# OpenVisualCloud/SVT-VP9

Measured on AMD Instinct MI355X. Metric: hot-path frames/sec (+ Mpixels/sec): block-level DSP path (picture analysis + ME + inter prediction from reconstructed references + DCT/quant/recon + deblock + reference padding), 3840x2160p60 yuv420p enc-mode 8; no mode decision, no entropy coding -- not encoded frames, higher is better.
Workload: dtype u8

## Files before the change

include/svtvp9_hip.h:

```cpp
#ifndef SVTVP9_HIP_H
#define SVTVP9_HIP_H

#include <stddef.h>
#include <stdint.h>

#ifdef __cplusplus
extern "C" {
#endif

typedef enum svt_hip_status {
    SVT_HIP_OK                 = 0,
    SVT_HIP_ERR_BAD_PARAMETER  = -1,
    SVT_HIP_ERR_NO_RESOURCES   = -2,
    SVT_HIP_ERR_DEVICE         = -3,
    SVT_HIP_ERR_UNSUPPORTED    = -4
} svt_hip_status;

typedef struct svt_hip_ctx svt_hip_ctx;


#define SVT_ME_PU_COUNT 85
#define SVT_SB_SIZE 64

typedef struct svt_plane {
// ... 54 lines not shown
    int16_t         x_mv_l0, y_mv_l0, x_mv_l1, y_mv_l1;
    svt_me_dist_dir distortion_direction[3];
    uint8_t         total_me_candidate_index;
    uint8_t         pad_[7];
} svt_me_pu_result;

int32_t svt_hip_sb_count(int32_t pic_width, int32_t pic_height);

int32_t svt_hip_input_resolution(int32_t pic_width, int32_t pic_height);

typedef struct svt_me_picture_config {
    int32_t pic_width, pic_height;
    int32_t enc_mode;
    int32_t tune;
    int32_t frame_rate;
    int32_t num_ref_lists;
    int32_t temporal_layer_index;
    int32_t hierarchical_levels;
    int32_t is_used_as_reference;
    int32_t same_ref_poc;
    int32_t rate_control_mode;
} svt_me_picture_config;

int32_t svt_hip_me_params_derive(svt_me_params *p, const svt_me_picture_config *cfg);

int32_t svt_hip_me_params_preset(svt_me_params *p, int32_t pic_width, int32_t pic_height, int32_t enc_mode,
                                 int32_t tune, int32_t num_ref_lists, int32_t temporal_layer_index,
                                 int32_t hierarchical_levels);

int32_t svt_hip_me_kernel_instance(const svt_me_params *p);
int32_t svt_hip_me_last_instance(const svt_hip_ctx *ctx);
int32_t svt_hip_me_lds_bytes(const svt_me_params *p, int32_t compact);
int32_t svt_hip_ctx_set_intra_workgroups(svt_hip_ctx *ctx, int32_t n);
int32_t svt_hip_ctx_warm(svt_hip_ctx *ctx);
int32_t svt_hip_ctx_warm_scratch(svt_hip_ctx *ctx, int32_t scratch_bytes);
int32_t svt_hip_me_params_same_launch(const svt_me_params *a, const svt_me_params *b);

int32_t svt_hip_ctx_create(svt_hip_ctx **ctx, int32_t device_ordinal);
int32_t svt_hip_ctx_create_on_stream(svt_hip_ctx **ctx, int32_t device_ordinal, void *hip_stream);
int32_t svt_hip_ctx_create_cu_mask(svt_hip_ctx **ctx, int32_t device, const uint32_t *cu_mask, int32_t mask_words);
void *svt_hip_ctx_stream(svt_hip_ctx *ctx);
void    svt_hip_ctx_destroy(svt_hip_ctx *ctx);
int32_t svt_hip_ctx_synchronize(svt_hip_ctx *ctx);
const char *svt_hip_last_error(void);
float   svt_hip_last_kernel_ms(svt_hip_ctx *ctx);

int32_t svt_hip_mem_alloc(svt_hip_ctx *ctx, size_t bytes, void **d_ptr);
void    svt_hip_mem_free(svt_hip_ctx *ctx, void *d_ptr);
int32_t svt_hip_mem_upload_2d(svt_hip_ctx *ctx, void *d_dst, size_t dst_stride, const void *src, size_t src_stride, size_t width_bytes,
                              size_t rows);
int32_t svt_hip_mem_download(svt_hip_ctx *ctx, void *dst, const void *d_src, size_t bytes);
int32_t svt_hip_mem_upload_2d_async(svt_hip_ctx *ctx, void *d_dst, size_t dst_stride, const void *src, size_t src_stride, size_t width_bytes,
                                    size_t rows);
int32_t svt_hip_mem_upload_planes_async(svt_hip_ctx *ctx, int32_t n_planes, void *const *d_dst, const size_t *dst_stride, const void *const *src,
                                        const size_t *src_stride, const size_t *width_bytes, const size_t *rows);
int32_t svt_hip_mem_upload_2d_direct(svt_hip_ctx *ctx, void *d_dst, size_t dst_stride, const void *src, size_t src_stride, size_t width_bytes,
                                     size_t rows);
int32_t svt_hip_mem_upload_wait(svt_hip_ctx *ctx);
void    svt_hip_host_unregister_all(void);
void    svt_hip_host_registry_retain(void);
void    svt_hip_host_registry_release(void);
int32_t svt_hip_ctx_marker_record(svt_hip_ctx *ctx, uint64_t *marker);
int32_t svt_hip_ctx_marker_query(svt_hip_ctx *ctx, uint64_t marker);
int32_t svt_hip_ctx_marker_wait(svt_hip_ctx *ctx, uint64_t marker);
int32_t svt_hip_mem_set(svt_hip_ctx *ctx, void *d_dst, int32_t value, size_t bytes);

// ... 459 lines not shown
```

svt-vp9_amd/binding.py:

```python
import ctypes as C
import os

import numpy as np

HERE = os.path.dirname(os.path.abspath(__file__))
LIB_PATH = os.environ.get("SVT_HIP_LIB") or os.path.join(HERE, "libsvtvp9_hip.so")

SVT_ME_PU_COUNT = 85


class Plane(C.Structure):
    _fields_ = [("buf", C.c_void_p), ("stride", C.c_int32), ("origin_x", C.c_int32), ("origin_y", C.c_int32),
                ("width", C.c_int32), ("height", C.c_int32)]


class PaPicture(C.Structure):
    _fields_ = [("full", Plane), ("quarter", Plane), ("sixteenth", Plane)]


class MeParams(C.Structure):
    _fields_ = [(n, C.c_uint8) for n in (
        "num_ref_lists", "temporal_layer_index", "hierarchical_levels", "enable_hme_flag",
        "enable_hme_level_0_flag", "enable_hme_level_1_flag", "enable_hme_level_2_flag", "cu8x8_mode",
        "cu16x16_mode", "same_ref_poc", "rate_control_mode", "fractional_search_method",
# ... 126 lines not shown
assert BOOL_TABLES_DTYPE.itemsize == 576 * 3 + 255 * 8 + 6 * 14
BOOL_SEGMENT_DTYPE = np.dtype([("first", "<u4"), ("count", "<u4"), ("kind", "<u4")])
BOOL_MAX_PER_TOKEN = 22
BOOL_SIZE_OVERFLOW = 0xFFFFFFFF
BOOL_MAX_STREAMS = 32


class BoolStream(C.Structure):
    _fields_ = [("d_tokens", C.c_void_p), ("d_bools", C.c_void_p), ("d_segments", C.c_void_p), ("d_n_tokens", C.c_void_p), ("n_segments", C.c_uint32),
                ("n_tokens", C.c_uint32), ("max_bools", C.c_uint32), ("capacity", C.c_uint32), ("d_bytes", C.c_void_p), ("d_size", C.c_void_p)]

OIS_BLOCK_DTYPE = np.dtype([("sad", "<u4"), ("uv_sad", "<u4"), ("mode", "u1"), ("uv_mode", "u1"), ("pad", "u1", (2,))])
assert OIS_BLOCK_DTYPE.itemsize == 12
OIS_PER_SB = 340
OIS_NONE = 0xFFFFFFFF

EXPORTS = [
    "svt_hip_sb_count", "svt_hip_input_resolution", "svt_hip_me_params_derive", "svt_hip_me_params_preset", "svt_hip_ctx_create", "svt_hip_ctx_create_on_stream", "svt_hip_ctx_create_cu_mask", "svt_hip_ctx_stream",
    "svt_hip_ctx_destroy", "svt_hip_ctx_synchronize", "svt_hip_last_error", "svt_hip_last_kernel_ms",
    "svt_hip_mem_alloc", "svt_hip_mem_free", "svt_hip_mem_upload_2d", "svt_hip_mem_upload_2d_async", "svt_hip_mem_upload_planes_async", "svt_hip_mem_download", "svt_hip_mem_set",
    "svt_hip_ctx_marker_record", "svt_hip_ctx_marker_query", "svt_hip_ctx_marker_wait", "svt_hip_minigop_split",
    "svt_hip_me_picture_device", "svt_hip_me_batch_device", "svt_hip_me_batch_layers_device", "svt_hip_me_picture", "svt_hip_sad_loop_batch_device",
    "svt_hip_me_zz_sad_device", "svt_hip_me_similar_collocated", "svt_hip_me_sb_stats_device", "svt_hip_pa_prepare_batch_device", "svt_hip_pa_mean_variance_device",
    "svt_hip_quant_tables_init", "svt_hip_tq_batch_device", "svt_hip_tq_batch_dist_device", "svt_hip_tq_rd_batch_device", "svt_hip_tq_rd_batch_multi_device", "svt_hip_rate_scan4x4_table", "svt_hip_tq_batch", "svt_hip_lf_thresh_init", "svt_hip_lf_level_from_q",
    "svt_hip_lf_frame_device", "svt_hip_lf_batch_device", "svt_hip_lf_frame", "svt_hip_lf_build_masks",
    "svt_hip_inter_pred_batch_device", "svt_hip_inter_pred_frame", "svt_hip_ref_pad_batch_device", "svt_hip_coeff_rate_batch_device", "svt_hip_coeff_rate_batch",
    "svt_hip_gop_owner", "svt_hip_gop_assign", "svt_hip_minigop_reference_source", "svt_hip_device_set_create", "svt_hip_device_set_size",
    "svt_hip_device_set_ctx", "svt_hip_device_set_destroy", "svt_hip_ref_handoff_device",
    "svt_ivf_stream_header", "svt_ivf_packetize",
    "svt_hip_tq_blocks_from_grid", "svt_hip_vp9_iscan_tables", "svt_hip_vp9_qindex_from_qp", "svt_hip_vp9_dc_step", "svt_hip_vp9_ac_step",
    "svt_hip_quant_tables_for_qindex", "svt_hip_encdec_flags_derive", "svt_hip_encdec_work_create", "svt_hip_encdec_work_destroy",
    "svt_hip_encdec_batch_device", "svt_hip_encdec_intra_device", "svt_hip_md_intra_default_device", "svt_hip_encdec_work_status", "svt_hip_encdec_work_download", "svt_hip_md_default_batch_device",
    "svt_hip_md_default_picture", "svt_hip_lf_build_masks_device", "svt_hip_ctx_wait_marker", "svt_hip_host_alloc", "svt_hip_host_free",
    "svt_hip_mem_download_2d_async", "svt_hip_mem_copy_2d_device", "svt_hip_encdec_work_set_stage_hook", "svt_hip_me_params_same_launch", "svt_hip_me_kernel_instance", "svt_hip_ctx_set_intra_workgroups", "svt_hip_ctx_warm", "svt_hip_ctx_warm_scratch", "svt_hip_lf_reserve",
    "svt_hip_me_last_instance", "svt_hip_me_lds_bytes", "svt_hip_vp9_layer_qindex", "svt_hip_mem_upload_2d_direct", "svt_hip_mem_upload_wait", "svt_hip_host_unregister_all", "svt_hip_host_registry_retain", "svt_hip_host_registry_release",
    "svt_hip_intra_search_device", "svt_hip_md_intra_search_device", "svt_hip_md_intra_search_picture",
    "svt_hip_pa_noise_params_derive", "svt_hip_pa_noise_batch_device", "svt_hip_pa_histogram_batch_device", "svt_hip_pa_chroma_mean_batch_device",
    "svt_hip_vp9_scan_tables", "svt_hip_tokenize_blocks_device", "svt_hip_tokenize_blocks", "svt_hip_tokenize_blocks_host", "svt_hip_tokenize_batch_device", "svt_hip_tokenize_picture",
    "svt_hip_tokenize_capacity",
    "svt_hip_boolcode_set_tables", "svt_hip_boolcode_batch_device", "svt_hip_boolcode", "svt_hip_boolcode_host", "svt_hip_boolcode_capacity", "svt_hip_boolcode_bools_capacity",
    "svt_hip_boolcode_geometry",
]

_lib = None


def load():
    global _lib
    if _lib is None:
        if not os.path.exists(LIB_PATH):
            raise RuntimeError(f"{LIB_PATH} not built: run `python -c 'import __graft_entry__ as g; g.build()'`")
        try:
            import torch
        except Exception:
            pass
        _lib = C.CDLL(LIB_PATH)
        _lib.svt_hip_last_error.restype = C.c_char_p
        _lib.svt_hip_ctx_stream.restype = C.c_void_p
        _lib.svt_hip_ctx_stream.argtypes = [C.c_void_p]
        _lib.svt_hip_last_kernel_ms.restype = C.c_float
        _lib.svt_hip_last_kernel_ms.argtypes = [C.c_void_p]
        _lib.svt_hip_lf_thresh_init.restype = None
        _lib.svt_hip_vp9_iscan_tables.restype = C.POINTER(C.c_int16)
        _lib.svt_hip_vp9_iscan_tables.argtypes = [C.POINTER(C.POINTER(C.c_uint32)), C.POINTER(C.c_int32)]
        _lib.svt_hip_vp9_scan_tables.restype = C.POINTER(C.c_int16)
        _lib.svt_hip_vp9_scan_tables.argtypes = [C.POINTER(C.POINTER(C.c_uint32)), C.POINTER(C.c_int32)]
        _lib.svt_hip_tokenize_capacity.restype = C.c_uint32
# ... 62 lines not shown
```

svt-vp9_amd/csrc/api.hip:

```cpp
#include <hip/hip_runtime.h>
#include <time.h>
#include <stdio.h>
#include <stdlib.h>
#include <string.h>
#include "svt_ctx.h"

extern "C" void svt_copy_rows_mt(uint8_t *dst, size_t dst_stride, const uint8_t *src, size_t src_stride, size_t width, size_t rows);
extern "C" void svt_copy_planes_mt(int n_planes, uint8_t *const *dst, const size_t *dst_stride, const uint8_t *const *src, const size_t *src_stride, const size_t *width,
                                   const size_t *rows);

static thread_local char g_err[512] = "";

int32_t svt_set_error(int32_t code, const char *msg) {
    snprintf(g_err, sizeof g_err, "%s", msg);
    return code;
}
int32_t svt_set_hip_error(hipError_t e, const char *file, int line) {
    snprintf(g_err, sizeof g_err, "HIP error %d (%s) at %s:%d", (int)e, hipGetErrorString(e), file, line);
    return SVT_HIP_ERR_DEVICE;
}
extern "C" const char *svt_hip_last_error(void) { return g_err; }

extern "C" int32_t svt_hip_sb_count(int32_t w, int32_t h) { return ((w + 63) / 64) * ((h + 63) / 64); }

// ... 41 lines not shown
extern "C" int32_t svt_hip_ctx_create(svt_hip_ctx **ctx, int32_t device) { return ctx_create(ctx, device, nullptr, 1); }
extern "C" int32_t svt_hip_ctx_create_on_stream(svt_hip_ctx **ctx, int32_t device, void *s) { return ctx_create(ctx, device, s, 0); }

extern "C" int32_t svt_hip_ctx_create_cu_mask(svt_hip_ctx **ctx, int32_t device, const uint32_t *cu_mask, int32_t mask_words) {
    if (!cu_mask || mask_words < 1) return svt_set_error(SVT_HIP_ERR_BAD_PARAMETER, "ctx: empty CU mask");
    return ctx_create(ctx, device, nullptr, 1, cu_mask, mask_words);
}
extern "C" void *svt_hip_ctx_stream(svt_hip_ctx *c) { return c ? (void *)c->stream : nullptr; }
template <int WORDS> __global__ void svt_ctx_warm_kernel(uint32_t *p, int n) {
    if constexpr (WORDS > 0) {
        volatile uint32_t a[WORDS];
        uint32_t          acc = 0;
        for (int i = 0; i < n && i < WORDS; i++) a[i] = (uint32_t)(i * n);
        for (int i = 0; i < n; i++) acc += a[(i * 7) % WORDS];
        if (p && n > 0) *p = acc;
    } else if (p && n > 0) *p = 0;
}
extern "C" int32_t svt_hip_ctx_warm_scratch(svt_hip_ctx *c, int32_t scratch_bytes) {
    if (!c || scratch_bytes < 0) return svt_set_error(SVT_HIP_ERR_BAD_PARAMETER, "ctx_warm: bad argument");
    HIP_TRY(hipSetDevice(c->device));
    uint32_t *p = (uint32_t *)c->ring_slab_dev;
    const dim3 grid((unsigned)(c->cu_count > 0 ? c->cu_count * 8 : 2048));
    if (scratch_bytes == 0) hipLaunchKernelGGL(svt_ctx_warm_kernel<0>, dim3(1), dim3(64), 0, c->stream, p, 0);
    else if (scratch_bytes <= 256) hipLaunchKernelGGL(svt_ctx_warm_kernel<64>, grid, dim3(64), 0, c->stream, p, 0);
    else hipLaunchKernelGGL(svt_ctx_warm_kernel<256>, grid, dim3(64), 0, c->stream, p, 0);
    HIP_TRY(hipGetLastError());
    HIP_TRY(hipStreamSynchronize(c->stream));
    return SVT_HIP_OK;
}
extern "C" int32_t svt_hip_ctx_warm(svt_hip_ctx *c) { return svt_hip_ctx_warm_scratch(c, 0); }
extern "C" int32_t svt_hip_ctx_set_intra_workgroups(svt_hip_ctx *c, int32_t n) {
    if (!c || n < 0) return svt_set_error(SVT_HIP_ERR_BAD_PARAMETER, "ctx: intra workgroups");
    c->intra_wgs = n;
    return SVT_HIP_OK;
}

extern "C" void svt_hip_ctx_destroy(svt_hip_ctx *c) {
    if (!c) return;
    (void)hipSetDevice(c->device);
    if (c->up_prof_n)
        fprintf(stderr, "svt_hip upload profile (us per picture): staging-slot wait %.1f  row copies %.1f  enqueue %.1f  (%ld uploads)\n", 1e6 * c->up_prof[0] / (double)c->up_prof_n,
                1e6 * c->up_prof[1] / (double)c->up_prof_n, 1e6 * c->up_prof[2] / (double)c->up_prof_n, c->up_prof_n);
    if (c->stream || !c->owns_stream) (void)hipStreamSynchronize(c->stream);
    for (int i = 0; i < SVT_CTX_SLOTS; i++) if (c->slot[i]) (void)hipFree(c->slot[i]);
    for (int i = 0; i < SVT_CTX_RING; i++) {
        if (c->ring_own[i]) {
            if (c->ring_dev[i]) (void)hipFree(c->ring_dev[i]);
            if (c->ring_host[i]) (void)hipHostFree(c->ring_host[i]);
        }
        if (c->ring_ev[i]) (void)hipEventDestroy(c->ring_ev[i]);
    }
    if (c->ring_slab_dev) (void)hipFree(c->ring_slab_dev);
    if (c->ring_slab_host) (void)hipHostFree(c->ring_slab_host);
    for (int i = 0; i < SVT_CTX_UPLOAD_RING; i++) {
        if (c->up_host[i]) (void)hipHostFree(c->up_host[i]);
        if (c->up_ev[i]) (void)hipEventDestroy(c->up_ev[i]);
        if (i == 0 && c->direct_ev) (void)hipEventDestroy(c->direct_ev);
    }
    for (int i = 0; i < SVT_CTX_MARKERS; i++) if (c->mk_ev[i]) (void)hipEventDestroy(c->mk_ev[i]);
    if (c->ho_produced) (void)hipEventDestroy(c->ho_produced);
    if (c->ho_consumed) (void)hipEventDestroy(c->ho_consumed);
    if (c->ev_start) (void)hipEventDestroy(c->ev_start);
    if (c->ev_stop) (void)hipEventDestroy(c->ev_stop);
    if (c->owns_stream && c->stream) (void)hipStreamDestroy(c->stream);
    free(c);
}
// ... 340 lines not shown
```

svt-vp9_amd/csrc/encdec.hip:

```cpp
#include <hip/hip_runtime.h>
#include <stdlib.h>
#include <string.h>
#include "svt_ctx.h"
#include "encdec_core.h"

#define ED_MAX_PICS 32
#define ED_MAX_SETS 8

struct svt_encdec_work {
    int           max_pics, width, height, n_sb, sb_cols, mi_rows, mi_cols;
    size_t        cap_per_pic;
    svt_tq_block *d_blocks;
    void         *last_hb;
    uint32_t     *d_pos;
    uint16_t     *d_eob;
    int32_t      *d_counts;
    int32_t      *d_totals, *d_bases;
    int32_t      *d_off_cnt;
    int32_t      *d_status;
    int32_t      *d_intra_sync;
    svt_quant_tables *d_qtabs;
    int16_t      *d_iscan;
    svt_encdec_stage_hook hook;
    void         *hook_user;
// ... 320 lines not shown
        for (int k = n_sets - 1; k >= 0 && set < 0; k--)
            if (r_lo >= (uintptr_t)recon_set[k] && (uint64_t)(r_hi - (uintptr_t)recon_set[k]) + plane_span < (1ull << 32)) set = k;
        if (set < 0) return svt_set_error(SVT_HIP_ERR_BAD_PARAMETER, "encdec: the batch's reconstruction buffers span more than 8 regions of 4 GB");
        svt_tq_pic_geom &g = P.g;
        const uint8_t *s3[3] = {p.src.y, p.src.u, p.src.v}, *p3[3] = {p.pred.y, p.pred.u, p.pred.v};
        for (int k = 0; k < 3; k++) {
            g.src_off[k] = (uint32_t)((uintptr_t)s3[k] - src_lo); g.pred_off[k] = (uint32_t)((uintptr_t)p3[k] - pred_lo);
            g.recon_off[k] = (uint32_t)((uintptr_t)r3[k] - (uintptr_t)recon_set[set]);
        }
        if (p.src.y_stride > 65535 || p.pred.y_stride > 65535 || p.recon.y_stride > 65535) return svt_set_error(SVT_HIP_ERR_BAD_PARAMETER, "encdec: stride");
        g.src_stride[0] = (uint16_t)p.src.y_stride; g.src_stride[1] = (uint16_t)p.src.uv_stride;
        g.pred_stride[0] = (uint16_t)p.pred.y_stride; g.pred_stride[1] = (uint16_t)p.pred.uv_stride;
        g.recon_stride[0] = (uint16_t)p.recon.y_stride; g.recon_stride[1] = (uint16_t)p.recon.uv_stride;
        g.coeff_base = (uint32_t)q_off; g.width = width; g.height = height; g.recon_set = (uint8_t)set; g.pic = (uint8_t)i; g.do_recon = flags->do_recon ? 1 : 0;
        mcp[i].d_mi = p.d_mc_mi; mcp[i].mi_stride = mi_stride; mcp[i].mi_rows = hb.mi_rows; mcp[i].mi_cols = hb.mi_cols;
        mcp[i].ref[0] = p.ref[0]; mcp[i].ref[1] = p.ref[1]; mcp[i].pred = p.pred; mcp[i].use_subpel = p.use_subpel;
        rec[i] = p.recon; rec[i].width = width; rec[i].height = height;
        if (!p.no_pad) rec_pad[n_rec_pad++] = rec[i];
        lfm[i] = p.d_lfm; lfm_stride[i] = hb.sb_cols; mi_rows_a[i] = hb.mi_rows; mi_cols_a[i] = hb.mi_cols;
    }
    const ed_batch_dev *dB = nullptr;
    if (stage_batch(ctx, hb, &dB)) return svt_set_error(SVT_HIP_ERR_NO_RESOURCES, "encdec: descriptor buffers");
    {
        svt_quant_tables qt[2];
        if (svt_hip_quant_tables_for_qindex(q_index, qt) != SVT_HIP_OK) return svt_set_error(SVT_HIP_ERR_BAD_PARAMETER, "encdec: q index");
        void *h = nullptr, *d = nullptr;
        if (svt_ctx_stage(ctx, sizeof qt, &h, &d)) return svt_set_error(SVT_HIP_ERR_NO_RESOURCES, "encdec: descriptor buffers");
        memcpy(h, qt, sizeof qt);
        HIP_TRY(hipMemcpyAsync(w->d_qtabs, h, sizeof qt, hipMemcpyHostToDevice, ctx->stream));
        svt_ctx_stage_commit(ctx);
    }
#define ED_STAGE(k) do { if (w->hook) w->hook(w->hook_user, (k)); } while (0)
    ED_STAGE(SVT_ENCDEC_STAGE_MC);
    int32_t rc = svt_hip_inter_pred_batch_device(ctx, n_pics, mcp);
    if (rc) return rc;
    ED_STAGE(SVT_ENCDEC_STAGE_LISTS);
    const int nwg = n_pics * hb.n_sb;
    hipLaunchKernelGGL(svt_tq_count_kernel, dim3(nwg), dim3(64), 0, ctx->stream, dB, w->d_counts, w->d_status);
    hipLaunchKernelGGL(svt_scan_sb_kernel, dim3(4 * n_pics), dim3(256), 0, ctx->stream, w->d_counts, hb.n_sb, w->d_totals);
    hipLaunchKernelGGL(svt_scan_pic_kernel, dim3(1), dim3(64), 0, ctx->stream, (const int32_t *)w->d_totals, n_pics, w->d_bases, w->d_off_cnt);
    hipLaunchKernelGGL(svt_tq_emit_kernel, dim3(nwg), dim3(64), 0, ctx->stream, dB, (const int32_t *)w->d_counts, (const int32_t *)w->d_bases, (svt_tq_block *)nullptr, w->d_pos);
    HIP_TRY(hipGetLastError());
    if (!w->last_hb) w->last_hb = malloc(sizeof hb);
    if (w->last_hb) memcpy(w->last_hb, &hb, sizeof hb);
    ED_STAGE(SVT_ENCDEC_STAGE_TQ);
    int32_t cap[4];
    for (int s = 0; s < 4; s++) cap[s] = (int32_t)((size_t)n_pics * width * height * 3 / 2 / (size_t)(16 << (2 * s)));
    rc = svt_tq_launch_device_lists(ctx, (const uint8_t *)src_lo, (const uint8_t *)pred_lo, recon_set, n_sets, nullptr, cap, w->d_off_cnt, w->d_qtabs, w->d_iscan,
                                    (int16_t *)q_lo, (int16_t *)dq_lo, w->d_eob, nullptr, w->d_pos, &dB->pic[0].g, (int)sizeof(ed_pic_dev), dB->iscan_off, hb.sb_cols);
    if (rc) return rc;
    ED_STAGE(SVT_ENCDEC_STAGE_SKIP);
    {
        const size_t map_bytes = (size_t)(width / 4) * (height / 4) * 3 / 2 * sizeof(uint16_t);
        uintptr_t    low = map_bytes;
        for (int i = 0; i < n_pics; i++) low |= (uintptr_t)pics[i].d_eob_map;
        if (!(low & 15))
            hipLaunchKernelGGL(svt_eob_map_clear_kernel, dim3(64, n_pics), dim3(256), 0, ctx->stream, dB, (int)(map_bytes / 16));
        else
            for (int i = 0; i < n_pics; i++) HIP_TRY(hipMemsetAsync(pics[i].d_eob_map, 0, map_bytes, ctx->stream));
    }
    for (int i = 0; i < n_pics; i++)
        if (pics[i].has_intra) {
            if (!flags->do_recon) return svt_set_error(SVT_HIP_ERR_BAD_PARAMETER, "encdec: intra blocks need the reconstruction (do_recon)");
            rc = svt_intra_launch(ctx, &pics[i], width, height, mi_stride, w->d_qtabs, w->d_iscan, hb.iscan_off, w->d_intra_sync, w->d_status, 1);
            if (rc) return rc;
        }
    {
// ... 183 lines not shown
```

svt-vp9_amd/csrc/mc_kernel.hip:

```cpp
#include <hip/hip_runtime.h>
#include "svt_ctx.h"

namespace {

struct mc_pic_dev {
    const svt_mc_mode_info *mi;
    int32_t        mi_stride, mi_rows, mi_cols;
    svt_yuv_planes ref[2];
    svt_yuv_planes pred;
    int32_t        use_subpel;
};

#define PK(a, b, c, d) ((uint32_t)(uint8_t)(int8_t)(a) | (uint32_t)(uint8_t)(int8_t)(b) << 8 | (uint32_t)(uint8_t)(int8_t)(c) << 16 | (uint32_t)(uint8_t)(int8_t)(d) << 24)
__constant__ uint32_t c_tap_lo[16] = {PK(0, 0, 0, 0), PK(0, 1, -5, 126), PK(-1, 3, -10, 122), PK(-1, 4, -13, 118), PK(-1, 4, -16, 112), PK(-1, 5, -18, 105),
                                      PK(-1, 5, -19, 97), PK(-1, 6, -19, 88), PK(-1, 6, -19, 78), PK(-1, 5, -18, 68), PK(-1, 5, -16, 58), PK(-1, 4, -14, 48),
                                      PK(-1, 4, -11, 37), PK(-1, 3, -9, 27), PK(0, 2, -6, 18), PK(0, 1, -3, 8)};
__constant__ uint32_t c_tap_hi[16] = {PK(0, 0, 0, 0), PK(8, -3, 1, 0), PK(18, -6, 2, 0), PK(27, -9, 3, -1), PK(37, -11, 4, -1), PK(48, -14, 4, -1),
                                      PK(58, -16, 5, -1), PK(68, -18, 5, -1), PK(78, -19, 6, -1), PK(88, -19, 6, -1), PK(97, -19, 5, -1), PK(105, -18, 5, -1),
                                      PK(112, -16, 4, -1), PK(118, -13, 4, -1), PK(122, -10, 3, -1), PK(126, -5, 1, 0)};

typedef uint32_t u32x4a4 __attribute__((ext_vector_type(4), aligned(4)));

__device__ __forceinline__ uint32_t alignbyte(uint32_t hi, uint32_t lo, uint32_t sh) { return __builtin_amdgcn_alignbyte(hi, lo, sh); }
__device__ __forceinline__ int clampi(int v, int lo, int hi) { return v < lo ? lo : v > hi ? hi : v; }
__device__ __forceinline__ uint32_t finish(int acc) { return (uint32_t)clampi(acc >> 7, 0, 255); }
__device__ __forceinline__ int dot4_bias(uint32_t a, uint32_t b, int bias) {
    int r;
    __asm__("v_dot4_i32_i8 %0, %1, %2, %3" : "=v"(r) : "v"(a), "v"(b), "s"(bias));
    return r;
}
__device__ __forceinline__ uint32_t pack4(uint32_t a, uint32_t b, uint32_t c, uint32_t d) {
    return __builtin_amdgcn_perm(c | (d << 8), a | (b << 8), 0x05040100u);
}
// ... 22 lines not shown
        const int      bias = 128 * 128 + 64;
        int            a0 = __builtin_amdgcn_sdot4((int)b1, (int)th, dot4_bias(b0, tl, bias), false);
        int            a1 = __builtin_amdgcn_sdot4((int)alignbyte(b2, b1, 1), (int)th, dot4_bias(alignbyte(b1, b0, 1), tl, bias), false);
        int            a2 = __builtin_amdgcn_sdot4((int)alignbyte(b2, b1, 2), (int)th, dot4_bias(alignbyte(b1, b0, 2), tl, bias), false);
        int            a3 = __builtin_amdgcn_sdot4((int)alignbyte(b2, b1, 3), (int)th, dot4_bias(alignbyte(b1, b0, 3), tl, bias), false);
        const uint32_t f = pack4(finish(a0), finish(a1), finish(a2), finish(a3));
        mid[r] = sx ? f : alignbyte(e1, e0, 3);
    }
    if (!any_sy) {
        _Pragma("unroll") for (int yy = 0; yy < NR; yy++) out[yy] = mid[yy + 3];
        return;
    }
    uint32_t col[4][NG];
    _Pragma("unroll") for (int g = 0; g < NG; g++) {
        const uint32_t r0 = mid[4 * g] ^ 0x80808080u, r1 = mid[4 * g + 1] ^ 0x80808080u, r2 = mid[4 * g + 2] ^ 0x80808080u;
        const uint32_t r3 = 4 * g + 3 < NM ? mid[4 * g + 3] ^ 0x80808080u : 0u;
        const uint32_t a0 = __builtin_amdgcn_perm(r1, r0, 0x05010400u), a1 = __builtin_amdgcn_perm(r1, r0, 0x07030602u);
        const uint32_t q0 = __builtin_amdgcn_perm(r3, r2, 0x05010400u), q1 = __builtin_amdgcn_perm(r3, r2, 0x07030602u);
        col[0][g] = __builtin_amdgcn_perm(q0, a0, 0x05040100u); col[1][g] = __builtin_amdgcn_perm(q0, a0, 0x07060302u);
        col[2][g] = __builtin_amdgcn_perm(q1, a1, 0x05040100u); col[3][g] = __builtin_amdgcn_perm(q1, a1, 0x07060302u);
    }
    const uint32_t vl = c_tap_lo[sy], vh = c_tap_hi[sy];
    _Pragma("unroll") for (int yy = 0; yy < NR; yy++) {
        uint32_t o[4];
        const int g0 = yy >> 2, sft = yy & 3;
        _Pragma("unroll") for (int j = 0; j < 4; j++) {
            const uint32_t lo = sft ? alignbyte(col[j][g0 + 1], col[j][g0], sft) : col[j][g0], hi = sft ? alignbyte(col[j][g0 + 2], col[j][g0 + 1], sft) : col[j][g0 + 1];
            o[j] = finish(__builtin_amdgcn_sdot4((int)hi, (int)vh, dot4_bias(lo, vl, 128 * 128 + 64), false));
        }
        out[yy] = sy ? pack4(o[0], o[1], o[2], o[3]) : mid[yy + 3];
    }
}

template <int NR>
__device__ __forceinline__ void mc_unit(const mc_pic_dev &P, int plane, int mi_row, int mi_col, int x, int y) {
    const uint32_t MC_GLOBAL *mp = MC_AS_GLOBAL(const uint32_t, P.mi + (size_t)mi_row * P.mi_stride + mi_col);
    const uint32_t  m0 = mp[0], m1 = mp[1], m2 = mp[2];
    const int       rl0 = (int8_t)(m2 & 0xff), rl1 = (int8_t)((m2 >> 8) & 0xff), bw8 = (int)((m2 >> 16) & 0xff), bh8 = (int)(m2 >> 24);
    if (rl0 < 0 || bw8 < 1 || bh8 < 1) return;
    const int ss = plane ? 1 : 0;
    const int bc = mi_col - mi_col % bw8, br = mi_row - mi_row % bh8;
    const int to_left = -(bc * 64), to_right = (P.mi_cols - bw8 - bc) * 64, to_top = -(br * 64), to_bottom = (P.mi_rows - bh8 - br) * 64;
    const int bw = (bw8 * 8) >> ss, bh = (bh8 * 8) >> ss;
    const int spel_left = (4 + bw) << 4, spel_right = spel_left - 16, spel_top = (4 + bh) << 4, spel_bottom = spel_top - 16;
    const int sc = 1 << (1 - ss);
    uint32_t  acc[NR];
    const int nref = rl1 >= 0 ? 2 : 1;
    for (int k = 0; k < nref; k++) {
        const svt_yuv_planes &R = P.ref[(k ? rl1 : rl0) ? 1 : 0];
        int mv_row = (int16_t)(k ? m0 >> 16 : m0 & 0xffff) * sc, mv_col = (int16_t)(k ? m1 >> 16 : m1 & 0xffff) * sc;
        mv_col = clampi(mv_col, to_left * sc - spel_left, to_right * sc + spel_right);
        mv_row = clampi(mv_row, to_top * sc - spel_top, to_bottom * sc + spel_bottom);
        int s_row, s_col, sx, sy;
        if (P.use_subpel) { s_row = mv_row; s_col = mv_col; sx = s_col & 15; sy = s_row & 15; }
        else if (plane) { s_row = (mv_row + 4) & ~7; s_col = (mv_col + 4) & ~7; sx = s_col & 7; sy = s_row & 7; }
        else { s_row = (mv_row + 8) & ~15; s_col = (mv_col + 8) & ~15; sx = s_col & 15; sy = s_row & 15; }
        const uint8_t *pl = plane == 0 ? R.y : plane == 1 ? R.u : R.v;
        uint32_t       o[NR];
        mc_tile<NR>(pl, plane ? R.uv_stride : R.y_stride, x, y, s_row, s_col, sx, sy, o);
        _Pragma("unroll") for (int r = 0; r < NR; r++)
            acc[r] = k ? __builtin_amdgcn_lerp(acc[r], o[r], 0x01010101u) : o[r];
    }
    uint8_t  *dp = plane == 0 ? P.pred.y : plane == 1 ? P.pred.u : P.pred.v;
    const int ds = plane ? P.pred.uv_stride : P.pred.y_stride;
    _Pragma("unroll") for (int r = 0; r < NR; r++) *MC_AS_GLOBAL(uint32_t, dp + (size_t)(y + r) * ds + x) = acc[r];
}

__global__ __launch_bounds__(128) void svt_mc_kernel(const mc_pic_dev *__restrict__ pics, int max_rows, int xblocks, int total, int chunk) {
    const int item = (int)(blockIdx.x & 7) * chunk + (int)(blockIdx.x >> 3);
    if (item >= total) return;
    const int xb = item % xblocks, rowpic = item / xblocks, mi_row = rowpic % max_rows;
    const mc_pic_dev &P = pics[rowpic / max_rows];
    const int t = threadIdx.x, wave = t >> 6, lane = t & 63;
    if (mi_row >= P.mi_rows) return;
    if (wave == 0) {
        const int mi_col = xb * 32 + (lane >> 1);
        if (mi_col < P.mi_cols) mc_unit<8>(P, 0, mi_row, mi_col, mi_col * 8 + 4 * (lane & 1), mi_row * 8);
    } else {
        const int mi_col = xb * 32 + (lane & 31);
        if (mi_col < P.mi_cols) mc_unit<4>(P, 1 + (lane >> 5), mi_row, mi_col, mi_col * 4, mi_row * 4);
    }
}

int mc_launch(svt_hip_ctx *ctx, int n_pics, const svt_mc_picture *pics) {
    int max_rows = 0, max_cols = 0;
    for (int i = 0; i < n_pics; i++) {
        const svt_mc_picture &p = pics[i];
        if (!p.d_mi || p.mi_rows < 1 || p.mi_cols < 1 || p.mi_stride < p.mi_cols || !p.pred.y || !p.pred.u || !p.pred.v)
            return svt_set_error(SVT_HIP_ERR_BAD_PARAMETER, "mc: bad picture descriptor");
        for (int l = 0; l < 2; l++)
            if (!p.ref[l].y || !p.ref[l].u || !p.ref[l].v) return svt_set_error(SVT_HIP_ERR_BAD_PARAMETER, "mc: both reference lists need planes");
        if (((uintptr_t)p.pred.y | (uintptr_t)p.pred.u | (uintptr_t)p.pred.v | (uintptr_t)p.pred.y_stride | (uintptr_t)p.pred.uv_stride) & 3)
            return svt_set_error(SVT_HIP_ERR_BAD_PARAMETER, "mc: prediction planes and strides must be multiples of 4 bytes");
        max_rows = p.mi_rows > max_rows ? p.mi_rows : max_rows;
        max_cols = p.mi_cols > max_cols ? p.mi_cols : max_cols;
    }
    mc_pic_dev *h = nullptr, *d = nullptr;
    if (svt_ctx_stage(ctx, sizeof(mc_pic_dev) * (size_t)n_pics, (void **)&h, (void **)&d)) return svt_set_error(SVT_HIP_ERR_NO_RESOURCES, "mc: scratch");
    for (int i = 0; i < n_pics; i++) {
        h[i].mi = pics[i].d_mi; h[i].mi_stride = pics[i].mi_stride; h[i].mi_rows = pics[i].mi_rows; h[i].mi_cols = pics[i].mi_cols;
        h[i].ref[0] = pics[i].ref[0]; h[i].ref[1] = pics[i].ref[1]; h[i].pred = pics[i].pred; h[i].use_subpel = pics[i].use_subpel;
    }
    HIP_TRY(hipMemcpyAsync(d, h, sizeof(mc_pic_dev) * (size_t)n_pics, hipMemcpyHostToDevice, ctx->stream));
    HIP_TRY(hipEventRecord(ctx->ev_start, ctx->stream));
    const int xblocks = (max_cols + 31) / 32, total = xblocks * max_rows * n_pics, chunk = (total + 7) / 8;
    hipLaunchKernelGGL(svt_mc_kernel, dim3(chunk * 8), dim3(128), 0, ctx->stream, (const mc_pic_dev *)d, max_rows, xblocks, total, chunk);
    HIP_TRY(hipGetLastError());
    HIP_TRY(hipEventRecord(ctx->ev_stop, ctx->stream));
    svt_ctx_stage_commit(ctx);
    ctx->timed = 1;
    return SVT_HIP_OK;
}
}

extern "C" int32_t svt_hip_inter_pred_batch_device(svt_hip_ctx *ctx, int32_t n_pics, const svt_mc_picture *pics) {
    if (!ctx || n_pics < 1 || !pics) return svt_set_error(SVT_HIP_ERR_BAD_PARAMETER, "mc: null argument");
    HIP_TRY(hipSetDevice(ctx->device));
    return mc_launch(ctx, n_pics, pics);
}

extern "C" int32_t svt_hip_inter_pred_frame(svt_hip_ctx *ctx, const svt_mc_mode_info *mi, int32_t mi_stride, int32_t mi_rows, int32_t mi_cols,
                                            const svt_mc_host_ref ref[2], int32_t use_subpel, uint8_t *pred_y, uint8_t *pred_u, uint8_t *pred_v) {
    if (!ctx || !mi || !ref || !pred_y || !pred_u || !pred_v || mi_rows < 1 || mi_cols < 1 || mi_stride < mi_cols)
        return svt_set_error(SVT_HIP_ERR_BAD_PARAMETER, "mc: null argument");
    HIP_TRY(hipSetDevice(ctx->device));
    const int      W = mi_cols * 8, H = mi_rows * 8;
    svt_mc_picture p;
    memset(&p, 0, sizeof p);
    const size_t mi_bytes = sizeof(svt_mc_mode_info) * (size_t)mi_rows * mi_stride;
    void        *dmi      = svt_ctx_slot(ctx, 26, mi_bytes);
    if (!dmi) return svt_set_error(SVT_HIP_ERR_NO_RESOURCES, "mc: device buffers");
    HIP_TRY(hipMemcpyAsync(dmi, mi, mi_bytes, hipMemcpyHostToDevice, ctx->stream));
    p.d_mi = (const svt_mc_mode_info *)dmi; p.mi_stride = mi_stride; p.mi_rows = mi_rows; p.mi_cols = mi_cols; p.use_subpel = use_subpel;
    for (int l = 0; l < 2; l++) {
        const svt_mc_host_ref &r = ref[l];
        if (!r.y || !r.u || !r.v || r.org_x < 80 || r.org_y < 80 || (r.org_x & 1) || (r.org_y & 1))
            return svt_set_error(SVT_HIP_ERR_BAD_PARAMETER, "mc: reference planes need an even padding of at least 80 luma samples");
        const size_t ny = (size_t)r.y_stride * (H + 2 * r.org_y), nuv = (size_t)r.uv_stride * (H / 2 + r.org_y);
        uint8_t *dy = (uint8_t *)svt_ctx_slot(ctx, 27 + 3 * l, ny + 64);
        uint8_t *du = (uint8_t *)svt_ctx_slot(ctx, 28 + 3 * l, nuv + 64), *dv = (uint8_t *)svt_ctx_slot(ctx, 29 + 3 * l, nuv + 64);
        if (!dy || !du || !dv) return svt_set_error(SVT_HIP_ERR_NO_RESOURCES, "mc: device buffers");
        HIP_TRY(hipMemcpyAsync(dy, r.y, ny, hipMemcpyHostToDevice, ctx->stream));
        HIP_TRY(hipMemcpyAsync(du, r.u, nuv, hipMemcpyHostToDevice, ctx->stream));
        HIP_TRY(hipMemcpyAsync(dv, r.v, nuv, hipMemcpyHostToDevice, ctx->stream));
        p.ref[l].y = dy + (size_t)r.org_y * r.y_stride + r.org_x;
        p.ref[l].u = du + (size_t)(r.org_y / 2) * r.uv_stride + r.org_x / 2;
        p.ref[l].v = dv + (size_t)(r.org_y / 2) * r.uv_stride + r.org_x / 2;
        p.ref[l].y_stride = r.y_stride; p.ref[l].uv_stride = r.uv_stride; p.ref[l].width = W; p.ref[l].height = H;
    }
    const size_t ysz = (size_t)W * H, csz = ysz / 4;
    uint8_t     *dp  = (uint8_t *)svt_ctx_slot(ctx, 33, ysz + 2 * csz);
    if (!dp) return svt_set_error(SVT_HIP_ERR_NO_RESOURCES, "mc: device buffers");
    HIP_TRY(hipMemcpyAsync(dp, pred_y, ysz, hipMemcpyHostToDevice, ctx->stream));
    HIP_TRY(hipMemcpyAsync(dp + ysz, pred_u, csz, hipMemcpyHostToDevice, ctx->stream));
    HIP_TRY(hipMemcpyAsync(dp + ysz + csz, pred_v, csz, hipMemcpyHostToDevice, ctx->stream));
    p.pred.y = dp; p.pred.u = dp + ysz; p.pred.v = dp + ysz + csz; p.pred.y_stride = W; p.pred.uv_stride = W / 2; p.pred.width = W; p.pred.height = H;
    int32_t rc = mc_launch(ctx, 1, &p);
    if (rc) return rc;
    HIP_TRY(hipMemcpyAsync(pred_y, dp, ysz, hipMemcpyDeviceToHost, ctx->stream));
    HIP_TRY(hipMemcpyAsync(pred_u, dp + ysz, csz, hipMemcpyDeviceToHost, ctx->stream));
    HIP_TRY(hipMemcpyAsync(pred_v, dp + ysz + csz, csz, hipMemcpyDeviceToHost, ctx->stream));
    HIP_TRY(hipStreamSynchronize(ctx->stream));
    return SVT_HIP_OK;
}
```

svt-vp9_amd/csrc/svt_ctx.h:

```cpp
#ifndef SVT_CTX_H
#define SVT_CTX_H
#include <hip/hip_runtime.h>
#include <stdint.h>
#include <string.h>
#include "../../include/svtvp9_hip.h"

#define SVT_CTX_SLOTS 50
#define SVT_CTX_RING 64
#define SVT_CTX_UPLOAD_RING 4
#define SVT_CTX_MARKERS 1024

struct svt_hip_ctx {
    int         device;
    hipStream_t stream;
    int         owns_stream;
    hipEvent_t  ev_start, ev_stop;
    int         timed;
    int         cu_count;
    int         me_instance;
    int         intra_wgs;
    void       *ring_host[SVT_CTX_RING];
    void       *ring_dev[SVT_CTX_RING];
    size_t      ring_bytes[SVT_CTX_RING];
    hipEvent_t  ring_ev[SVT_CTX_RING];
    int         ring_used[SVT_CTX_RING];
    int         ring_own[SVT_CTX_RING];
    void       *ring_slab_host, *ring_slab_dev;
    int         ring_pos;
    void       *up_host[SVT_CTX_UPLOAD_RING];
    size_t      up_bytes[SVT_CTX_UPLOAD_RING];
    hipEvent_t  up_ev[SVT_CTX_UPLOAD_RING];
    int         up_used[SVT_CTX_UPLOAD_RING];
    int         up_pos;
    double      up_prof[3];
    long        up_prof_n;
    hipEvent_t  direct_ev;
    int         direct_pending;
    hipEvent_t  mk_ev[SVT_CTX_MARKERS];
    uint64_t    mk_next;
    hipEvent_t  ho_produced, ho_consumed;
    void       *slot[SVT_CTX_SLOTS];
    size_t      slot_bytes[SVT_CTX_SLOTS];
};

int32_t svt_set_error(int32_t code, const char *msg);
int32_t svt_set_hip_error(hipError_t e, const char *file, int line);
int     svt_ctx_stage(svt_hip_ctx *ctx, size_t bytes, void **host, void **dev);
void    svt_ctx_stage_commit(svt_hip_ctx *ctx);
void   *svt_ctx_slot(svt_hip_ctx *ctx, int slot, size_t bytes);

int32_t svt_tq_launch_device_lists(svt_hip_ctx *ctx, const uint8_t *d_src, const uint8_t *d_pred, uint8_t *const *recon_set, int n_set,
                                   const svt_tq_block *d_blocks, const int32_t cap[4], const int32_t *d_off_cnt, const svt_quant_tables *d_qtabs,
                                   const int16_t *d_iscan, int16_t *d_qcoeff, int16_t *d_dqcoeff, uint16_t *d_eob, uint64_t *d_dist,
                                   const uint32_t *d_pos, const void *d_geom, int geom_stride, const uint32_t *d_iscan_off, int sb_cols);

int32_t svt_intra_launch(svt_hip_ctx *ctx, const svt_encdec_picture *p, int32_t width, int32_t height, int32_t mi_stride, const svt_quant_tables *d_qtabs,
                         const int16_t *d_iscan, const uint32_t iscan_off[16], int32_t *d_sync, int32_t *d_status, int32_t mixed);
int32_t svt_md_intra_default_launch(svt_hip_ctx *ctx, svt_lf_mode_info *d_lf_mi, int32_t mi_stride, int32_t mi_rows, int32_t mi_cols, int32_t filter_level);

#define HIP_TRY(expr)                                                        \
    do {                                                                     \
        hipError_t e_ = (expr);                                              \
        if (e_ != hipSuccess) return svt_set_hip_error(e_, __FILE__, __LINE__); \
    } while (0)
#endif
```

Before: 6744.

## Make inter-prediction kernel persistent with banded work walk and mode-info prefetch

The motion-compensation kernel changes from one 128-thread workgroup per row-chunk to a capped grid of 256-thread persistent workgroups. Each workgroup strides through banded pairs of items, alternating luma and chroma roles per wave, and prefetches the next item's mode-info words while computing the current one. Grid size comes from CU count, with a context setter and an environment override. This aims to cut launch and tail overhead and hide mode-info load latency, at the cost of more register pressure and possible load imbalance across bands.

```diff
diff --git a/include/svtvp9_hip.h b/include/svtvp9_hip.h
--- a/include/svtvp9_hip.h
+++ b/include/svtvp9_hip.h
@@ -110,6 +110,7 @@
 int32_t svt_hip_me_last_instance(const svt_hip_ctx *ctx);
 int32_t svt_hip_me_lds_bytes(const svt_me_params *p, int32_t compact);
 int32_t svt_hip_ctx_set_intra_workgroups(svt_hip_ctx *ctx, int32_t n);
+int32_t svt_hip_ctx_set_mc_workgroups(svt_hip_ctx *ctx, int32_t n);
 int32_t svt_hip_ctx_warm(svt_hip_ctx *ctx);
 int32_t svt_hip_ctx_warm_scratch(svt_hip_ctx *ctx, int32_t scratch_bytes);
 int32_t svt_hip_me_params_same_launch(const svt_me_params *a, const svt_me_params *b);
diff --git a/svt-vp9_amd/binding.py b/svt-vp9_amd/binding.py
--- a/svt-vp9_amd/binding.py
+++ b/svt-vp9_amd/binding.py
@@ -182,7 +182,7 @@
     "svt_hip_quant_tables_for_qindex", "svt_hip_encdec_flags_derive", "svt_hip_encdec_work_create", "svt_hip_encdec_work_destroy",
     "svt_hip_encdec_batch_device", "svt_hip_encdec_intra_device", "svt_hip_md_intra_default_device", "svt_hip_encdec_work_status", "svt_hip_encdec_work_download", "svt_hip_md_default_batch_device",
     "svt_hip_md_default_picture", "svt_hip_lf_build_masks_device", "svt_hip_ctx_wait_marker", "svt_hip_host_alloc", "svt_hip_host_free",
-    "svt_hip_mem_download_2d_async", "svt_hip_mem_copy_2d_device", "svt_hip_encdec_work_set_stage_hook", "svt_hip_me_params_same_launch", "svt_hip_me_kernel_instance", "svt_hip_ctx_set_intra_workgroups", "svt_hip_ctx_warm", "svt_hip_ctx_warm_scratch", "svt_hip_lf_reserve",
+    "svt_hip_mem_download_2d_async", "svt_hip_mem_copy_2d_device", "svt_hip_encdec_work_set_stage_hook", "svt_hip_me_params_same_launch", "svt_hip_me_kernel_instance", "svt_hip_ctx_set_intra_workgroups", "svt_hip_ctx_set_mc_workgroups", "svt_hip_ctx_warm", "svt_hip_ctx_warm_scratch", "svt_hip_lf_reserve",
     "svt_hip_me_last_instance", "svt_hip_me_lds_bytes", "svt_hip_vp9_layer_qindex", "svt_hip_mem_upload_2d_direct", "svt_hip_mem_upload_wait", "svt_hip_host_unregister_all", "svt_hip_host_registry_retain", "svt_hip_host_registry_release",
     "svt_hip_intra_search_device", "svt_hip_md_intra_search_device", "svt_hip_md_intra_search_picture",
     "svt_hip_pa_noise_params_derive", "svt_hip_pa_noise_batch_device", "svt_hip_pa_histogram_batch_device", "svt_hip_pa_chroma_mean_batch_device",
diff --git a/svt-vp9_amd/csrc/api.hip b/svt-vp9_amd/csrc/api.hip
--- a/svt-vp9_amd/csrc/api.hip
+++ b/svt-vp9_amd/csrc/api.hip
@@ -97,6 +97,11 @@
 extern "C" int32_t svt_hip_ctx_set_intra_workgroups(svt_hip_ctx *c, int32_t n) {
     if (!c || n < 0) return svt_set_error(SVT_HIP_ERR_BAD_PARAMETER, "ctx: intra workgroups");
     c->intra_wgs = n;
+    return SVT_HIP_OK;
+}
+extern "C" int32_t svt_hip_ctx_set_mc_workgroups(svt_hip_ctx *c, int32_t n) {
+    if (!c || n < 0) return svt_set_error(SVT_HIP_ERR_BAD_PARAMETER, "ctx: inter-prediction workgroups");
+    c->mc_wgs = n;
     return SVT_HIP_OK;
 }
 
diff --git a/svt-vp9_amd/csrc/encdec.hip b/svt-vp9_amd/csrc/encdec.hip
--- a/svt-vp9_amd/csrc/encdec.hip
+++ b/svt-vp9_amd/csrc/encdec.hip
@@ -376,7 +376,7 @@
     }
 #define ED_STAGE(k) do { if (w->hook) w->hook(w->hook_user, (k)); } while (0)
     ED_STAGE(SVT_ENCDEC_STAGE_MC);
-    int32_t rc = svt_hip_inter_pred_batch_device(ctx, n_pics, mcp);
+    int32_t rc = svt_mc_launch_encode_pass(ctx, n_pics, mcp);
     if (rc) return rc;
     ED_STAGE(SVT_ENCDEC_STAGE_LISTS);
     const int nwg = n_pics * hb.n_sb;
diff --git a/svt-vp9_amd/csrc/mc_kernel.hip b/svt-vp9_amd/csrc/mc_kernel.hip
--- a/svt-vp9_amd/csrc/mc_kernel.hip
+++ b/svt-vp9_amd/csrc/mc_kernel.hip
@@ -1,4 +1,5 @@
 #include <hip/hip_runtime.h>
+#include <stdlib.h>
 #include "svt_ctx.h"
 
 namespace {
@@ -87,10 +88,9 @@
     }
 }
 
+#define MC_NO_UNIT 0xffu
 template <int NR>
-__device__ __forceinline__ void mc_unit(const mc_pic_dev &P, int plane, int mi_row, int mi_col, int x, int y) {
-    const uint32_t MC_GLOBAL *mp = MC_AS_GLOBAL(const uint32_t, P.mi + (size_t)mi_row * P.mi_stride + mi_col);
-    const uint32_t  m0 = mp[0], m1 = mp[1], m2 = mp[2];
+__device__ __forceinline__ void mc_unit(const mc_pic_dev &P, int plane, int mi_row, int mi_col, int x, int y, uint32_t m0, uint32_t m1, uint32_t m2) {
     const int       rl0 = (int8_t)(m2 & 0xff), rl1 = (int8_t)((m2 >> 8) & 0xff), bw8 = (int)((m2 >> 16) & 0xff), bh8 = (int)(m2 >> 24);
     if (rl0 < 0 || bw8 < 1 || bh8 < 1) return;
     const int ss = plane ? 1 : 0;
@@ -121,23 +121,73 @@
     _Pragma("unroll") for (int r = 0; r < NR; r++) *MC_AS_GLOBAL(uint32_t, dp + (size_t)(y + r) * ds + x) = acc[r];
 }
 
-__global__ __launch_bounds__(128) void svt_mc_kernel(const mc_pic_dev *__restrict__ pics, int max_rows, int xblocks, int total, int chunk) {
-    const int item = (int)(blockIdx.x & 7) * chunk + (int)(blockIdx.x >> 3);
-    if (item >= total) return;
-    const int xb = item % xblocks, rowpic = item / xblocks, mi_row = rowpic % max_rows;
-    const mc_pic_dev &P = pics[rowpic / max_rows];
-    const int t = threadIdx.x, wave = t >> 6, lane = t & 63;
-    if (mi_row >= P.mi_rows) return;
-    if (wave == 0) {
-        const int mi_col = xb * 32 + (lane >> 1);
-        if (mi_col < P.mi_cols) mc_unit<8>(P, 0, mi_row, mi_col, mi_col * 8 + 4 * (lane & 1), mi_row * 8);
-    } else {
-        const int mi_col = xb * 32 + (lane & 31);
-        if (mi_col < P.mi_cols) mc_unit<4>(P, 1 + (lane >> 5), mi_row, mi_col, mi_col * 4, mi_row * 4);
-    }
-}
-
-int mc_launch(svt_hip_ctx *ctx, int n_pics, const svt_mc_picture *pics) {
+#ifndef MC_WALK_PREFETCH
+#define MC_WALK_PREFETCH 1
+#endif
+
+struct mc_item { int pic, mi_row, xb; bool ok; };
+
+__global__ __launch_bounds__(256) void svt_mc_kernel(const mc_pic_dev *__restrict__ pics, int max_rows, int xblocks, int total) {
+    const int wave = __builtin_amdgcn_readfirstlane((int)(threadIdx.x >> 6)), lane = (int)(threadIdx.x & 63);
+    const int npairs = (total + 1) >> 1, G = (int)gridDim.x, nb = G < 8 ? G : 8;
+    const int band = (int)blockIdx.x % nb, per_band = (npairs + nb - 1) / nb, base = band * per_band;
+    const int step = (G - band + nb - 1) / nb;
+    auto item_of = [&](int j) {
+        mc_item it;
+        const int item = 2 * (base + j) + (wave & 1), rowpic = item / xblocks;
+        it.ok = j < per_band && item < total;
+        it.xb = item - rowpic * xblocks; it.pic = rowpic / max_rows; it.mi_row = rowpic - it.pic * max_rows;
+        return it;
+    };
+    auto mi_load = [&](const mc_item &it, bool luma, int lane, uint32_t &m0, uint32_t &m1, uint32_t &m2) {
+        m0 = 0u; m1 = 0u; m2 = MC_NO_UNIT;
+        if (!it.ok) return;
+        const mc_pic_dev &P = pics[it.pic];
+        const int         mi_col = it.xb * 32 + (luma ? lane >> 1 : lane & 31);
+        if (it.mi_row < P.mi_rows && mi_col < P.mi_cols) {
+            const uint32_t MC_GLOBAL *mp = MC_AS_GLOBAL(const uint32_t, P.mi + (size_t)it.mi_row * P.mi_stride + mi_col);
+            m0 = mp[0]; m1 = mp[1]; m2 = mp[2];
+        }
+    };
+    int      j = (int)blockIdx.x / nb;
+    bool     luma = !(wave & 2);
+    mc_item  cur = item_of(j);
+    uint32_t m0, m1, m2;
+    mi_load(cur, luma, lane, m0, m1, m2);
+    while (j < per_band && base + j < npairs) {
+        const mc_item nxt = item_of(j + step);
+        uint32_t      n0, n1, n2;
+        int ln = lane;
+        __asm__ volatile("" : "+v"(ln));
+        if (MC_WALK_PREFETCH) mi_load(nxt, !luma, ln, n0, n1, n2);
+        if (cur.ok) {
+            const mc_pic_dev &P = pics[cur.pic];
+            if (luma) {
+                const int mi_col = cur.xb * 32 + (ln >> 1);
+                mc_unit<8>(P, 0, cur.mi_row, mi_col, mi_col * 8 + 4 * (ln & 1), cur.mi_row * 8, m0, m1, m2);
+            } else {
+                const int mi_col = cur.xb * 32 + (ln & 31);
+                mc_unit<4>(P, 1 + (ln >> 5), cur.mi_row, mi_col, mi_col * 4, cur.mi_row * 4, m0, m1, m2);
+            }
+        }
+        if (!MC_WALK_PREFETCH) mi_load(nxt, !luma, ln, n0, n1, n2);
+        m0 = n0; m1 = n1; m2 = n2;
+        cur = nxt; luma = !luma; j += step;
+    }
+}
+
+constexpr int MC_PER_2CU = 10, MC_PER_2CU_ENC = 10;
+
+int mc_grid(svt_hip_ctx *ctx, int npairs, int per_2cu) {
+    static const int env = [] { const char *e = getenv("SVT_HIP_MC_GRID"); return e ? atoi(e) : 0; }();
+    const int forced = ctx->mc_wgs > 0 ? ctx->mc_wgs : env;
+    if (forced > 0) return forced;
+    const int per_band = (npairs + 7) / 8, cap = (ctx->cu_count * per_2cu + 15) / 16;
+    const int trips = (per_band + cap - 1) / cap;
+    return 8 * ((per_band + trips - 1) / trips);
+}
+
+int mc_launch(svt_hip_ctx *ctx, int n_pics, const svt_mc_picture *pics, int per_2cu) {
     int max_rows = 0, max_cols = 0;
     for (int i = 0; i < n_pics; i++) {
         const svt_mc_picture &p = pics[i];
@@ -158,8 +208,8 @@
     }
     HIP_TRY(hipMemcpyAsync(d, h, sizeof(mc_pic_dev) * (size_t)n_pics, hipMemcpyHostToDevice, ctx->stream));
     HIP_TRY(hipEventRecord(ctx->ev_start, ctx->stream));
-    const int xblocks = (max_cols + 31) / 32, total = xblocks * max_rows * n_pics, chunk = (total + 7) / 8;
-    hipLaunchKernelGGL(svt_mc_kernel, dim3(chunk * 8), dim3(128), 0, ctx->stream, (const mc_pic_dev *)d, max_rows, xblocks, total, chunk);
+    const int xblocks = (max_cols + 31) / 32, total = xblocks * max_rows * n_pics;
+    hipLaunchKernelGGL(svt_mc_kernel, dim3(mc_grid(ctx, (total + 1) / 2, per_2cu)), dim3(256), 0, ctx->stream, (const mc_pic_dev *)d, max_rows, xblocks, total);
     HIP_TRY(hipGetLastError());
     HIP_TRY(hipEventRecord(ctx->ev_stop, ctx->stream));
     svt_ctx_stage_commit(ctx);
@@ -171,7 +221,13 @@
 extern "C" int32_t svt_hip_inter_pred_batch_device(svt_hip_ctx *ctx, int32_t n_pics, const svt_mc_picture *pics) {
     if (!ctx || n_pics < 1 || !pics) return svt_set_error(SVT_HIP_ERR_BAD_PARAMETER, "mc: null argument");
     HIP_TRY(hipSetDevice(ctx->device));
-    return mc_launch(ctx, n_pics, pics);
+    return mc_launch(ctx, n_pics, pics, MC_PER_2CU);
+}
+
+int32_t svt_mc_launch_encode_pass(svt_hip_ctx *ctx, int32_t n_pics, const svt_mc_picture *pics) {
+    if (!ctx || n_pics < 1 || !pics) return svt_set_error(SVT_HIP_ERR_BAD_PARAMETER, "mc: null argument");
+    HIP_TRY(hipSetDevice(ctx->device));
+    return mc_launch(ctx, n_pics, pics, MC_PER_2CU_ENC);
 }
 
 extern "C" int32_t svt_hip_inter_pred_frame(svt_hip_ctx *ctx, const svt_mc_mode_info *mi, int32_t mi_stride, int32_t mi_rows, int32_t mi_cols,
@@ -210,7 +266,7 @@
     HIP_TRY(hipMemcpyAsync(dp + ysz, pred_u, csz, hipMemcpyHostToDevice, ctx->stream));
     HIP_TRY(hipMemcpyAsync(dp + ysz + csz, pred_v, csz, hipMemcpyHostToDevice, ctx->stream));
     p.pred.y = dp; p.pred.u = dp + ysz; p.pred.v = dp + ysz + csz; p.pred.y_stride = W; p.pred.uv_stride = W / 2; p.pred.width = W; p.pred.height = H;
-    int32_t rc = mc_launch(ctx, 1, &p);
+    int32_t rc = mc_launch(ctx, 1, &p, MC_PER_2CU);
     if (rc) return rc;
     HIP_TRY(hipMemcpyAsync(pred_y, dp, ysz, hipMemcpyDeviceToHost, ctx->stream));
     HIP_TRY(hipMemcpyAsync(pred_u, dp + ysz, csz, hipMemcpyDeviceToHost, ctx->stream));
diff --git a/svt-vp9_amd/csrc/svt_ctx.h b/svt-vp9_amd/csrc/svt_ctx.h
--- a/svt-vp9_amd/csrc/svt_ctx.h
+++ b/svt-vp9_amd/csrc/svt_ctx.h
@@ -19,6 +19,7 @@
     int         cu_count;
     int         me_instance;
     int         intra_wgs;
+    int         mc_wgs;
     void       *ring_host[SVT_CTX_RING];
     void       *ring_dev[SVT_CTX_RING];
     size_t      ring_bytes[SVT_CTX_RING];
@@ -54,6 +55,8 @@
                                    const int16_t *d_iscan, int16_t *d_qcoeff, int16_t *d_dqcoeff, uint16_t *d_eob, uint64_t *d_dist,
                                    const uint32_t *d_pos, const void *d_geom, int geom_stride, const uint32_t *d_iscan_off, int sb_cols);
 
+int32_t svt_mc_launch_encode_pass(svt_hip_ctx *ctx, int32_t n_pics, const svt_mc_picture *pics);
+
 int32_t svt_intra_launch(svt_hip_ctx *ctx, const svt_encdec_picture *p, int32_t width, int32_t height, int32_t mi_stride, const svt_quant_tables *d_qtabs,
                          const int16_t *d_iscan, const uint32_t iscan_off[16], int32_t *d_sync, int32_t *d_status, int32_t mixed);
 int32_t svt_md_intra_default_launch(svt_hip_ctx *ctx, svt_lf_mode_info *d_lf_mi, int32_t mi_stride, int32_t mi_rows, int32_t mi_cols, int32_t filter_level);
```

Measured after the change: 6659. -1.3%, worse.
